# SZU-AdvTech-2022/232-Hierarchical-Density-based-Clustering-Using-Mapreduce

Hardware: AMD Instinct MI355X
Metric: points/sec end-to-end + mutual-reach distance evals/sec at 1/2/4/8 GPUs (higher is better)
Workload: dtype f64

## Files before the change

232-hierarchical-density-based-clustering-using-mapreduce_amd/csrc/flat.hip:

```cpp
#include <rocprim/device/device_scan.hpp>

#include <algorithm>
#include <chrono>
#include <numeric>

#include "common.hpp"
#include "internal.hpp"
#include "sort.hpp"
#include "ssort.hpp"

namespace hdb {

namespace {

constexpr int32_t NONE = INT32_MAX;
enum : int { FE_RANGE = 1, FE_NAN = 2, FE_CYCLE = 4, FE_ISOLATED = 8, FE_ROOTS = 16, FE_JUMP = 32 };

__device__ __forceinline__ uint32_t uf_prio(int32_t x, int64_t n) {
    uint32_t h = (uint32_t)x * 0x9E3779B1u;
    h ^= h >> 16;
    h *= 0x85EBCA6Bu;
    h ^= h >> 13;
    return (x >= n ? 0x80000000u : 0u) | (h >> 1);
}

struct __align__(16) LRec {
    int32_t uf, rootedge, csize, cmin;
};

__device__ __forceinline__ int32_t uf_ld(const int32_t *p) {
    return __hip_atomic_load(p, __ATOMIC_RELAXED, __HIP_MEMORY_SCOPE_AGENT);
}
__device__ __forceinline__ void uf_st(int32_t *p, int32_t v) {
    __hip_atomic_store(p, v, __ATOMIC_RELAXED, __HIP_MEMORY_SCOPE_AGENT);
}
__device__ __forceinline__ int32_t uf_find(LRec *lr, int32_t x) {
    int32_t *u = &lr->uf;
    while (true) {
        int32_t p = uf_ld(u + 4 * (int64_t)x);
        if (p == x) return x;
        int32_t g = uf_ld(u + 4 * (int64_t)p);
        if (g == p) return p;
        uf_st(u + 4 * (int64_t)x, g);
        x = g;
    }
}

__device__ __forceinline__ int32_t uf_unite(LRec *uf, int32_t a, int32_t b, int64_t n) {
    while (true) {
// ... 113 lines not shown
__global__ void fl_relabel_orig(const int32_t *__restrict__ pparent, const int32_t *__restrict__ eb, int64_t n,
                                int32_t *__restrict__ orig) {
    HDB_GRID_STRIDE(v, n) {
        const int32_t p = pparent[v];
        if (p == NONE) continue;
        orig[2 * (int64_t)p + (eb[p] == (int32_t)v ? 1 : 0)] = (int32_t)v;
    }
}
__global__ void fl_relabel(const int32_t *__restrict__ ea, const int32_t *__restrict__ eb,
                           const int32_t *__restrict__ pparent, int64_t m, int32_t *__restrict__ lab) {
    HDB_GRID_STRIDE(r, m) {
#pragma unroll
        for (int s = 0; s < 2; s++) {
            const int32_t v = s ? eb[r] : ea[r];
            const int32_t p = pparent[v];
            lab[2 * r + s] = 2 * p + (eb[p] == v ? 1 : 0);
        }
    }
}

__device__ __forceinline__ int64_t l_rank(int64_t i, int b) {
    return ((i >> b) << (b + 1)) | (i & ((int64_t(1) << b) - 1));
}

struct DC {
    int32_t *lab;
    LRec *lr;
    int32_t *stamp;
    int32_t *hooked;
    int32_t *parent;
    int32_t *esize;
    int32_t *eminid;
    const int32_t *orig;
    int64_t n, m;
};
__device__ __forceinline__ int32_t vid(const DC &c, int32_t x) { return c.orig ? c.orig[x] : x; }

__global__ void dc_init(DC c, int b, int j, int64_t nl) {
    HDB_GRID_STRIDE(i, nl) {
        int64_t r = l_rank(i, b);
        if (r >= c.m) continue;
#pragma unroll
        for (int s = 0; s < 2; s++) {
            int32_t x = c.lab[2 * r + s];
            c.lr[x] = LRec{x, -1, 0, NONE};
            c.stamp[x] = 2 * j;
        }
    }
}

__global__ void dc_unite(DC c, int b, int64_t nl, int *__restrict__ err) {
    HDB_GRID_STRIDE(i, nl) {
        int64_t r = l_rank(i, b);
        if (r >= c.m) continue;
        const int32_t h = uf_unite(c.lr, c.lab[2 * r], c.lab[2 * r + 1], c.n);
        c.hooked[r] = h;
        if (h < 0) atomicOr(err, FE_CYCLE);
    }
}

__device__ __forceinline__ int32_t wave_max(int32_t v) {
    for (int o = 32; o >= 1; o >>= 1) v = max(v, __shfl_xor(v, o));
    return v;
}
__device__ __forceinline__ int32_t wave_min(int32_t v) {
    for (int o = 32; o >= 1; o >>= 1) v = min(v, __shfl_xor(v, o));
    return v;
}
__device__ __forceinline__ int32_t wave_sum(int32_t v) {
    for (int o = 32; o >= 1; o >>= 1) v += __shfl_xor(v, o);
    return v;
}

constexpr int ROOT_TB = 256, ROOT_SLOTS = 512;
template <int TB, int SLOTS>
__global__ __launch_bounds__(TB) void dc_root(DC c, int b, int j, int64_t nl) {
    __shared__ int32_t skey[SLOTS], smax[SLOTS], ssum[SLOTS], smin[SLOTS];
    const int t = threadIdx.x;
    for (int64_t base = (int64_t)blockIdx.x * TB; base < nl; base += (int64_t)gridDim.x * TB) {
        for (int k = t; k < SLOTS; k += TB) {
            skey[k] = -1;
            smax[k] = -1;
            ssum[k] = 0;
            smin[k] = NONE;
        }
        __syncthreads();
        const int64_t i = base + t;
        const int64_t r = i < nl ? l_rank(i, b) : c.m;
        if (r < c.m) {
            const int32_t rep = uf_find(c.lr, c.lab[2 * r]);
            const int32_t x = c.hooked[r];
            c.hooked[r] = rep;
            const int32_t sz = x < 0 ? 0 : (x < c.n ? 1 : c.esize[x - c.n]);
            const int32_t mi = x < 0 ? NONE : (x < c.n ? vid(c, x) : c.eminid[x - c.n]);
            uint32_t h = uf_prio(rep, 0) & (SLOTS - 1);
            while (true) {
                int32_t k = atomicCAS(&skey[h], -1, rep);
                if (k == -1 || k == rep) break;
                h = (h + 1) & (SLOTS - 1);
            }
            atomicMax(&smax[h], (int32_t)r);
            if (sz) atomicAdd(&ssum[h], sz);
            if (mi != NONE) atomicMin(&smin[h], mi);
        }
        __syncthreads();
        for (int k = t; k < SLOTS; k += TB) {
            const int32_t rep = skey[k];
            if (rep < 0) continue;
            atomicMax(&c.lr[rep].rootedge, smax[k]);
            if (ssum[k]) atomicAdd(&c.lr[rep].csize, ssum[k]);
            if (smin[k] != NONE) atomicMin(&c.lr[rep].cmin, smin[k]);
        }
        __syncthreads();
    }
}

template <int TB, int SLOTS, int EPT>
__global__ __launch_bounds__(TB) void dc_root_multi(DC c, int b, int j, int64_t nl) {
    __shared__ int32_t skey[SLOTS], smax[SLOTS], ssum[SLOTS], smin[SLOTS];
    __shared__ int s_used;
    const int t = threadIdx.x;
    auto clear = [&]() {
        for (int k = t; k < SLOTS; k += TB) {
            skey[k] = -1;
            smax[k] = -1;
            ssum[k] = 0;
            smin[k] = NONE;
        }
        if (t == 0) s_used = 0;
    };
    auto flush = [&]() {
        for (int k = t; k < SLOTS; k += TB) {
            const int32_t rep = skey[k];
            if (rep < 0) continue;
            atomicMax(&c.lr[rep].rootedge, smax[k]);
            if (ssum[k]) atomicAdd(&c.lr[rep].csize, ssum[k]);
            if (smin[k] != NONE) atomicMin(&c.lr[rep].cmin, smin[k]);
        }
    };
    const int64_t per = (int64_t)TB * EPT;
    for (int64_t base = (int64_t)blockIdx.x * per; base < nl; base += (int64_t)gridDim.x * per) {
        clear();
        __syncthreads();
        for (int e = 0; e < EPT; e++) {
            const int64_t i = base + (int64_t)e * TB + t;
            const int64_t r = i < nl ? l_rank(i, b) : c.m;
            if (r < c.m) {
                const int32_t rep = uf_find(c.lr, c.lab[2 * r]);
                const int32_t x = c.hooked[r];
                c.hooked[r] = rep;
                const int32_t sz = x < 0 ? 0 : (x < c.n ? 1 : c.esize[x - c.n]);
                const int32_t mi = x < 0 ? NONE : (x < c.n ? vid(c, x) : c.eminid[x - c.n]);
                uint32_t h = uf_prio(rep, 0) & (SLOTS - 1);
                while (true) {
                    const int32_t k = atomicCAS(&skey[h], -1, rep);
                    if (k == -1) {
                        atomicAdd(&s_used, 1);
                        break;
                    }
                    if (k == rep) break;
                    h = (h + 1) & (SLOTS - 1);
                }
                atomicMax(&smax[h], (int32_t)r);
                if (sz) atomicAdd(&ssum[h], sz);
                if (mi != NONE) atomicMin(&smin[h], mi);
            }
            __syncthreads();
            if (e + 1 < EPT && s_used > SLOTS / 2 - TB) {
                flush();
                __syncthreads();
                clear();
                __syncthreads();
            }
        }
        flush();
        __syncthreads();
    }
}

__global__ void dc_root_direct(DC c, int b, int j, int64_t nl) {
    HDB_GRID_STRIDE(i, nl) {
        const int64_t r = l_rank(i, b);
        if (r >= c.m) continue;
        const int32_t rep = uf_find(c.lr, c.lab[2 * r]);
        const int32_t x = c.hooked[r];
        c.hooked[r] = rep;
        atomicMax(&c.lr[rep].rootedge, (int32_t)r);
        if (x >= 0) {
            atomicAdd(&c.lr[rep].csize, x < c.n ? 1 : c.esize[x - c.n]);
            atomicMin(&c.lr[rep].cmin, x < c.n ? vid(c, x) : c.eminid[x - c.n]);
        }
    }
}

__global__ void dc_link(DC c, int b, int j, int64_t nl) {
    HDB_GRID_STRIDE(i, nl) {
        int64_t r = l_rank(i, b);
        if (r >= c.m) continue;
        {
            const int32_t rep = c.hooked[r];
            const LRec q = c.lr[rep];
            if (q.rootedge == (int32_t)r) {
                c.esize[r] = q.csize + (rep < c.n ? 1 : c.esize[rep - c.n]);
                c.eminid[r] = min(q.cmin, rep < c.n ? vid(c, rep) : c.eminid[rep - c.n]);
            }
        }
        const int64_t u = r | (int64_t(1) << b);
        if (u >= c.m) continue;
#pragma unroll
        for (int s = 0; s < 2; s++) {
            int32_t x = c.lab[2 * u + s];
            if (c.stamp[x] == 2 * j) {
                const int32_t R = c.lr[uf_find(c.lr, x)].rootedge;
                if (uf_ld(c.parent + R) > (int32_t)u) atomicMin(&c.parent[R], (int32_t)u);
                c.lab[2 * u + s] = (int32_t)(c.n + R);
            }
        }
    }
}

template <int TB, int SLOTS, int EPT>
__global__ __launch_bounds__(TB) void dc_link_multi(DC c, int b, int j, int64_t nl) {
    __shared__ int32_t skey[SLOTS], smin[SLOTS];
    __shared__ int s_used;
    const int t = threadIdx.x;
    auto clear = [&]() {
        for (int k = t; k < SLOTS; k += TB) {
            skey[k] = -1;
            smin[k] = INT32_MAX;
        }
        if (t == 0) s_used = 0;
    };
    auto flush = [&]() {
        for (int k = t; k < SLOTS; k += TB) {
            const int32_t R = skey[k];
            if (R < 0) continue;
            if (uf_ld(c.parent + R) > smin[k]) atomicMin(&c.parent[R], smin[k]);
        }
    };
    const int64_t per = (int64_t)TB * EPT;
    for (int64_t base = (int64_t)blockIdx.x * per; base < nl; base += (int64_t)gridDim.x * per) {
        clear();
        __syncthreads();
        for (int e = 0; e < EPT; e++) {
            const int64_t i = base + (int64_t)e * TB + t;
            const int64_t r = i < nl ? l_rank(i, b) : c.m;
            if (r < c.m) {
                {
                    const int32_t rep = c.hooked[r];
                    const LRec q = c.lr[rep];
                    if (q.rootedge == (int32_t)r) {
                        c.esize[r] = q.csize + (rep < c.n ? 1 : c.esize[rep - c.n]);
                        c.eminid[r] = min(q.cmin, rep < c.n ? vid(c, rep) : c.eminid[rep - c.n]);
                    }
                }
                const int64_t u = r | (int64_t(1) << b);
                if (u < c.m) {
#pragma unroll
                    for (int s = 0; s < 2; s++) {
                        const int32_t x = c.lab[2 * u + s];
                        if (c.stamp[x] == 2 * j) {
                            const int32_t R = c.lr[uf_find(c.lr, x)].rootedge;
                            uint32_t h = uf_prio(R, 0) & (SLOTS - 1);
                            while (true) {
                                const int32_t k = atomicCAS(&skey[h], -1, R);
                                if (k == -1) {
                                    atomicAdd(&s_used, 1);
                                    break;
                                }
                                if (k == R) break;
                                h = (h + 1) & (SLOTS - 1);
                            }
                            atomicMin(&smin[h], (int32_t)u);
                            c.lab[2 * u + s] = (int32_t)(c.n + R);
                        }
                    }
                }
            }
            __syncthreads();
            if (e + 1 < EPT && s_used > SLOTS / 2 - 2 * TB) {
                flush();
                __syncthreads();
                clear();
                __syncthreads();
            }
        }
// ... 34 lines not shown
            c.hooked[r] = h;
            if (h < 0) e_cyc = 1;
        }
        dc_phase_sync();
        {
            int32_t *skey = tab, *smax = tab + RS, *ssum = tab + 2 * RS, *smin = tab + 3 * RS;
            auto clear = [&]() {
                for (int k = t; k < RS; k += TB) {
                    skey[k] = -1;
                    smax[k] = -1;
                    ssum[k] = 0;
                    smin[k] = NONE;
                }
                if (t == 0) s_used = 0;
            };
            auto flush = [&]() {
                for (int k = t; k < RS; k += TB) {
                    const int32_t rep = skey[k];
                    if (rep < 0) continue;
                    atomicMax(&c.lr[rep].rootedge, smax[k]);
                    if (ssum[k]) atomicAdd(&c.lr[rep].csize, ssum[k]);
                    if (smin[k] != NONE) atomicMin(&c.lr[rep].cmin, smin[k]);
                }
            };
            clear();
            __syncthreads();
            for (int64_t base = i0; base < i1; base += TB) {
                const int64_t i = base + t;
                if (i < i1) {
                    const int64_t r = l_rank(i, b);
                    const int32_t rep = uf_find(c.lr, c.lab[2 * r]);
                    const int32_t x = c.hooked[r];
                    c.hooked[r] = rep;
                    const int32_t sz = x < 0 ? 0 : (x < c.n ? 1 : c.esize[x - c.n]);
                    const int32_t mi = x < 0 ? NONE : (x < c.n ? vid(c, x) : c.eminid[x - c.n]);
                    uint32_t h = uf_prio(rep, 0) & (RS - 1);
                    while (true) {
                        const int32_t k = atomicCAS(&skey[h], -1, rep);
                        if (k == -1) {
                            atomicAdd(&s_used, 1);
                            break;
                        }
                        if (k == rep) break;
                        h = (h + 1) & (RS - 1);
                    }
                    atomicMax(&smax[h], (int32_t)r);
                    if (sz) atomicAdd(&ssum[h], sz);
                    if (mi != NONE) atomicMin(&smin[h], mi);
                }
                __syncthreads();
                if (base + TB < i1 && s_used > RS / 2 - TB) {
                    flush();
                    __syncthreads();
                    clear();
                    __syncthreads();
                }
            }
            flush();
        }
        dc_phase_sync();
        {
            int32_t *skey = tab, *smin = tab + KS;
            auto clear = [&]() {
                for (int k = t; k < KS; k += TB) {
                    skey[k] = -1;
                    smin[k] = INT32_MAX;
                }
                if (t == 0) s_used = 0;
            };
            auto flush = [&]() {
                for (int k = t; k < KS; k += TB) {
                    const int32_t R = skey[k];
                    if (R < 0) continue;
                    if (uf_ld(c.parent + R) > smin[k]) atomicMin(&c.parent[R], smin[k]);
                }
            };
            clear();
            __syncthreads();
            for (int64_t base = i0; base < i1; base += TB) {
                const int64_t i = base + t;
                if (i < i1) {
                    const int64_t r = l_rank(i, b);
                    {
                        const int32_t rep = c.hooked[r];
                        const LRec q = c.lr[rep];
                        if (q.rootedge == (int32_t)r) {
                            c.esize[r] = q.csize + (rep < c.n ? 1 : c.esize[rep - c.n]);
                            c.eminid[r] = min(q.cmin, rep < c.n ? vid(c, rep) : c.eminid[rep - c.n]);
                        }
                    }
                    const int64_t u = r | half;
                    if (u < c.m) {
#pragma unroll
                        for (int s = 0; s < 2; s++) {
                            const int32_t x = c.lab[2 * u + s];
                            if (c.stamp[x] == 2 * j) {
                                const int32_t R = c.lr[uf_find(c.lr, x)].rootedge;
                                uint32_t h = uf_prio(R, 0) & (KS - 1);
                                while (true) {
                                    const int32_t k = atomicCAS(&skey[h], -1, R);
                                    if (k == -1) {
                                        atomicAdd(&s_used, 1);
                                        break;
                                    }
                                    if (k == R) break;
                                    h = (h + 1) & (KS - 1);
                                }
                                atomicMin(&smin[h], (int32_t)u);
                                c.lab[2 * u + s] = (int32_t)(c.n + R);
                            }
                        }
                    }
                }
                __syncthreads();
                if (base + TB < i1 && s_used > KS / 2 - 2 * TB) {
                    flush();
                    __syncthreads();
                    clear();
                    __syncthreads();
                }
            }
// ... 17 lines not shown
        if (g == p) return p;
        ((volatile int32_t *)uf)[x] = g;
        x = g;
    }
}

template <int LB, int TB>
__global__ __launch_bounds__(TB) void dc_block(DC c, int *__restrict__ err) {
    using P = DcBlk<LB>;
    __shared__ int32_t key[P::HS], bsz[P::HS], bmn[P::HS];
    __shared__ int32_t uf[P::NL], re[P::NL], cs[P::NL], cm[P::NL];
    __shared__ int8_t stp[P::NL];
    __shared__ int16_t lab[2 * P::B];
    __shared__ int32_t esz[P::B], emn[P::B], lpar[P::B];
    __shared__ int16_t hk[P::B], rp[P::B];
    __shared__ int s_err;
    const int t = threadIdx.x;
    for (int64_t lo = (int64_t)blockIdx.x * P::B; lo < c.m; lo += (int64_t)gridDim.x * P::B) {
        const int cnt = (int)(c.m - lo < P::B ? c.m - lo : P::B);
        for (int k = t; k < P::HS; k += TB) key[k] = -1;
        for (int k = t; k < P::NL; k += TB) stp[k] = -1;
        for (int k = t; k < P::B; k += TB) {
            esz[k] = -1;
            lpar[k] = INT32_MAX;
        }
        if (t == 0) s_err = 0;
        __syncthreads();
        for (int k = t; k < 2 * cnt; k += TB) {
            const int32_t x = c.lab[2 * lo + k];
            uint32_t h = uf_prio(x, 0) & (P::HS - 1);
            while (true) {
                const int32_t old = atomicCAS(&key[h], -1, x);
                if (old == -1) {
                    bsz[h] = x < c.n ? 1 : c.esize[x - c.n];
                    bmn[h] = x < c.n ? vid(c, x) : c.eminid[x - c.n];
                    break;
                }
                if (old == x) break;
                h = (h + 1) & (P::HS - 1);
            }
            lab[k] = (int16_t)h;
        }
        __syncthreads();
        for (int b = LB - 1; b >= 0; b--) {
            const int half = 1 << b, nl = (P::B >> 1);
            for (int i = t; i < nl; i += TB) {
                const int k = ((i >> b) << (b + 1)) | (i & (half - 1));
                if (k >= cnt) continue;
#pragma unroll
                for (int s = 0; s < 2; s++) {
                    const int x = lab[2 * k + s];
                    uf[x] = x;
                    re[x] = -1;
                    cs[x] = x < P::HS ? bsz[x] : esz[x - P::HS];
                    cm[x] = x < P::HS ? bmn[x] : emn[x - P::HS];
                    stp[x] = (int8_t)b;
                }
            }
            __syncthreads();
            for (int i = t; i < nl; i += TB) {
                const int k = ((i >> b) << (b + 1)) | (i & (half - 1));
                if (k >= cnt) continue;
                int32_t a = lab[2 * k], d = lab[2 * k + 1], hooked = -1;
                while (true) {
                    a = lds_find(uf, a);
                    d = lds_find(uf, d);
                    if (a == d) break;
                    const uint32_t pa = uf_prio(a, P::HS), pd = uf_prio(d, P::HS);
                    if (pa < pd || (pa == pd && a < d)) {
                        const int32_t tt = a;
                        a = d;
                        d = tt;
                    }
                    if (atomicCAS(&uf[d], d, a) == d) {
                        hooked = d;
                        break;
                    }
                }
                if (hooked < 0) s_err = 1;
                hk[k] = (int16_t)hooked;
            }
            __syncthreads();
            for (int i = t; i < nl; i += TB) {
                const int k = ((i >> b) << (b + 1)) | (i & (half - 1));
                if (k >= cnt) continue;
                const int32_t rep = lds_find(uf, lab[2 * k]);
                rp[k] = (int16_t)rep;
                atomicMax(&re[rep], k);
                const int32_t x = hk[k];
                if (x >= 0) {
                    atomicAdd(&cs[rep], cs[x]);
                    atomicMin(&cm[rep], cm[x]);
                }
            }
            __syncthreads();
            for (int i = t; i < nl; i += TB) {
                const int k = ((i >> b) << (b + 1)) | (i & (half - 1));
                if (k >= cnt) continue;
                const int32_t rep = rp[k];
                if (re[rep] == k) {
                    esz[k] = cs[rep];
                    emn[k] = cm[rep];
                }
                const int u = k | half;
                if (u >= cnt) continue;
#pragma unroll
                for (int s = 0; s < 2; s++) {
                    const int x = lab[2 * u + s];
                    if (stp[x] == (int8_t)b) {
                        const int32_t R = re[lds_find(uf, x)];
                        atomicMin(&lpar[R], u);
                        lab[2 * u + s] = (int16_t)(P::HS + R);
                    }
                }
            }
            __syncthreads();
        }
        for (int k = t; k < cnt; k += TB) {
            if (esz[k] >= 0) {
                c.esize[lo + k] = esz[k];
                c.eminid[lo + k] = emn[k];
            }
            if (lpar[k] != INT32_MAX) c.parent[lo + k] = (int32_t)(lo + lpar[k]);
        }
        if (t == 0 && s_err) atomicOr(err, FE_CYCLE);
        __syncthreads();
    }
}

constexpr int LOC_LOG = 8, LOC_EDGES = 1 << LOC_LOG, LOC_SLOTS = 4 * LOC_EDGES;
__global__ __launch_bounds__(64) void dc_local(DC c, int *__restrict__ err) {
    __shared__ int32_t key[LOC_SLOTS], lsz[LOC_SLOTS], lmn[LOC_SLOTS];
    __shared__ int16_t luf[LOC_SLOTS], lre[LOC_SLOTS];
    __shared__ int16_t le[2 * LOC_EDGES];
    const int lane = threadIdx.x;
    for (int64_t lo = (int64_t)blockIdx.x * LOC_EDGES; lo < c.m; lo += (int64_t)gridDim.x * LOC_EDGES) {
        const int cnt = (int)(c.m - lo < LOC_EDGES ? c.m - lo : LOC_EDGES);
        for (int k = lane; k < LOC_SLOTS; k += 64) key[k] = -1;
        __syncthreads();
        for (int k = lane; k < 2 * cnt; k += 64) {
            const int32_t x = c.lab[2 * lo + k];
            uint32_t h = uf_prio(x, 0) & (LOC_SLOTS - 1);
            while (true) {
                const int32_t old = atomicCAS(&key[h], -1, x);
                if (old == -1) {
                    luf[h] = (int16_t)h;
                    lre[h] = -1;
                    lsz[h] = x < c.n ? 1 : c.esize[x - c.n];
                    lmn[h] = x < c.n ? vid(c, x) : c.eminid[x - c.n];
                    break;
                }
                if (old == x) break;
                h = (h + 1) & (LOC_SLOTS - 1);
            }
            le[k] = (int16_t)h;
        }
        __syncthreads();
        if (lane == 0) {
            auto find = [&](int x) {
                while (luf[x] != x) {
                    const int g = luf[luf[x]];
                    luf[x] = (int16_t)g;
                    x = g;
                }
                return x;
            };
            for (int k = 0; k < cnt; k++) {
                int a = find(le[2 * k]), b = find(le[2 * k + 1]);
                if (a == b) {
                    atomicOr(err, FE_CYCLE);
                    break;
                }
                if (lre[a] >= 0) c.parent[lo + lre[a]] = (int32_t)(lo + k);
                if (lre[b] >= 0) c.parent[lo + lre[b]] = (int32_t)(lo + k);
                if (lsz[a] < lsz[b]) {
                    const int t = a;
                    a = b;
                    b = t;
                }
                luf[b] = (int16_t)a;
                lsz[a] += lsz[b];
                lmn[a] = min(lmn[a], lmn[b]);
                lre[a] = (int16_t)k;
                c.esize[lo + k] = lsz[a];
                c.eminid[lo + k] = lmn[a];
            }
        }
        __syncthreads();
    }
}

__global__ void fl_tie_up(const int32_t *__restrict__ parent, const double *__restrict__ ew, int64_t m,
                          int32_t *__restrict__ up, int *__restrict__ err) {
    int e = 0;
    HDB_GRID_STRIDE(r, m) {
        int32_t p = parent[r];
        up[r] = (p != NONE && ew[p] == ew[r]) ? p : (int32_t)r;
        if (p == NONE && r != m - 1) e |= FE_ROOTS;
    }
    if (e) atomicOr(err, e);
}

__global__ void fl_jump(int32_t *__restrict__ up, int64_t m, const int *__restrict__ flag_prev,
                        int *__restrict__ flag_next) {
    if (flag_prev && *flag_prev == 0) return;
    int ch = 0;
    HDB_GRID_STRIDE(r, m) {
        int32_t p = up[r];
        bool moved = false;
#pragma unroll 1
        for (int it = 0; it < 2; it++) {
            const int32_t g = up[p];
            if (g == p) break;
            p = up[g];
            moved = true;
        }
        if (moved) {
            up[r] = p;
            ch = 1;
        }
    }
    flag_or(flag_next, ch);
// ... 943 lines not shown
                cur = c0;
                if (bt[cur] <= eps) {
                    int j = 0;
                    int32_t last = cur;
                    while (j < J) {
                        const int32_t a = anc[j * stride + cur];
                        if (!(bt[a] <= eps)) break;
                        last = a;
                        j++;
                    }
                    for (int jj = j - 2; jj >= 0; jj--) {
                        const int32_t a = anc[jj * stride + last];
                        if (bt[a] <= eps) last = a;
                    }
                    cur = anc[last];
                }
                const double pl = point_level[y], ee = pl > eps ? pl : eps;
                sc = ee == 0.0 ? 0.0 : 1.0 - ord_dec(em[cur]) / ee;
            }
        }
        if (tree_label) tree_label[i] = cur;
        if (labels) labels[i] = near[cur];
        if (scores) scores[i] = sc;
    }
    flag_or(err, e);
}

inline size_t fz_layout(int64_t m) { return (size_t)m * 24 + (size_t)m * 8 + 192 * 4; }

void throw_tree_errors(int e) {
    if (e & FE_CYCLE) HDB_THROW(HDB_EINVAL, "flat labels: the edges contain a cycle");
    if (e & FE_ROOTS) HDB_THROW(HDB_EINVAL, "flat labels: the edges are not a spanning tree");
    if (e & FE_JUMP) HDB_THROW(HDB_EDEVICE, "flat labels: pointer jumping did not converge in its launch budget");
}

}

static void flat_device_impl(hdb_ctx *ctx, const int32_t *va, const int32_t *vb, const double *w, int64_t ne,
                             int64_t n, int32_t mcs, int32_t *labels, int64_t *n_clusters, double *scores,
                             double *noise, const ClusterTreeOut *tree = nullptr) {
    if (n <= 0) {
        if (n_clusters) *n_clusters = 0;
        if (tree) *tree->n_tree = 0;
        return;
    }
    if (mcs < 2) HDB_THROW(HDB_EINVAL, "flat labels: minClSize must be >= 2");
    if (n >= (int64_t(1) << 30)) HDB_THROW(HDB_EINVAL, "flat labels: too many points");
    if (ne < 0) HDB_THROW(HDB_EINVAL, "bad arguments");
    hipStream_t st = ctx->stream;
    KernelTimer tt(ctx, "flat_labels");
    const int64_t m = n - 1;
    int64_t *pin = pinned_words(ctx) + PINNED_WORDS - 8;
    const int64_t mm = std::max<int64_t>(m, 1);
    const bool relabel = ctx->flat_relabel && m >= 1 && flat_relabel_fits(m);
    const int64_t nv = relabel ? 2 * mm : n;

    int32_t *keep, *pos, *ca, *cb, *ea, *eb, *orig, *pparent;
    double *cw, *ew;
    int64_t *words;
    DC dc;
    carve(ctx, A_FLAT0, [&](Carver &cv) {
        keep = cv.take<int32_t>(ne), pos = cv.take<int32_t>(ne);
        ca = cv.take<int32_t>(mm), cb = cv.take<int32_t>(mm);
        cw = cv.take<double>(mm);
        words = cv.take<int64_t>(4);
        ea = cv.take<int32_t>(mm), eb = cv.take<int32_t>(mm);
        ew = cv.take<double>(mm);
        dc.lab = cv.take<int32_t>(2 * mm);
        dc.lr = cv.take<LRec>(nv + mm);
        dc.stamp = cv.take<int32_t>(nv + mm);
        orig = cv.take<int32_t>(nv);
        dc.hooked = cv.take<int32_t>(mm);
        dc.parent = cv.take<int32_t>(mm);
        dc.esize = cv.take<int32_t>(mm);
        dc.eminid = cv.take<int32_t>(mm);
        pparent = cv.take<int32_t>(n);
    });
    int64_t *m_dev = words;
    int *err = (int *)(words + 1), *flags = (int *)(words + 2);
    dc.n = nv;
    dc.m = m;
    dc.orig = relabel ? orig : nullptr;

    HIP_CHECK(hipMemsetAsync(words, 0, sizeof(int64_t) * 4, st));
    if (ne > 0) {
        if (ne > INT32_MAX) HDB_THROW(HDB_EINVAL, "too many edges");
        hipLaunchKernelGGL(fl_mark, dim3(grid_for(ne)), dim3(256), 0, st, va, vb, w, ne, n, keep, err);
        exclusive_sum(ctx, A_FLAT_TMP, keep, pos, ne);
        hipLaunchKernelGGL(fl_compact, dim3(grid_for(ne)), dim3(256), 0, st, va, vb, w, ne, keep, pos, m, ca, cb, cw,
                           m_dev);
        hipLaunchKernelGGL(fl_order, dim3((unsigned)std::min<int64_t>(grid_for(ne) / 4 + 1, 256)), dim3(1024), 0, st,
                           cw, m_dev, flags);
    }
    HIP_CHECK(hipMemcpyAsync(pin, words, sizeof(int64_t) * 3, hipMemcpyDeviceToHost, st));
    HIP_CHECK(hipStreamSynchronize(st));
    const int64_t m_got = pin[0];
    const int e0 = (int)pin[1], order = (int)pin[2];
    if (e0 & FE_RANGE) HDB_THROW(HDB_EINVAL, "flat labels: vertex id out of range");
    if (e0 & FE_NAN) HDB_THROW(HDB_EINVAL, "flat labels: NaN edge weight");
    if (m_got != m) HDB_THROW(HDB_EINVAL, "flat labels: the edges are not a spanning tree");
    if (m == 0) {
        if (labels) HIP_CHECK(hipMemsetAsync(labels, 0, sizeof(int32_t), st));
        if (scores) HIP_CHECK(hipMemsetAsync(scores, 0, sizeof(double), st));
        if (noise) HIP_CHECK(hipMemsetAsync(noise, 0, sizeof(double), st));
        if (n_clusters) *n_clusters = 0;
        if (tree) {
            *tree->n_tree = 1;
            if (tree->cap < 1) HDB_THROW(HDB_EINVAL, "cluster tree: capacity 0 is below the 1 clusters of the tree");
            hipLaunchKernelGGL(ct_single, dim3(1), dim3(64), 0, st, *tree);
            HIP_CHECK(hipGetLastError());
            HIP_CHECK(hipStreamSynchronize(st));
        }
        return;
    }
    const int g = grid_for(m);
    const int32_t *perm = nullptr;
    int desc = !(order & 1);
    if (desc == 0 && (order & 2)) {
        double *k1, *k2;
        int32_t *i1, *i2;
        carve(ctx, A_FLAT1, [&](Carver &cv) {
            k1 = cv.take<double>(m), k2 = cv.take<double>(m);
            i1 = cv.take<int32_t>(m), i2 = cv.take<int32_t>(m);
        });
        hipLaunchKernelGGL(fl_sort_keys, dim3(g), dim3(256), 0, st, cw, m, k1, i1);
        sort_pairs(ctx, A_FLAT_TMP, k1, k2, i1, i2, m, 0, 64);
        perm = i2;
    }
    hipLaunchKernelGGL(fl_rank, dim3(g), dim3(256), 0, st, ca, cb, cw, m, desc, perm, ea, eb, ew, dc.lab, dc.parent);
    hipLaunchKernelGGL(fill_i32, dim3(grid_for(nv + m)), dim3(256), 0, st, dc.stamp, nv + m, -1);
    hipLaunchKernelGGL(fill_i32, dim3(grid_for(n)), dim3(256), 0, st, pparent, n, NONE);
    hipLaunchKernelGGL(fl_point_parent, dim3(g), dim3(256), 0, st, ea, eb, m, pparent);
    if (relabel) {
        hipLaunchKernelGGL(fl_relabel_orig, dim3(grid_for(n)), dim3(256), 0, st, pparent, eb, n, orig);
        hipLaunchKernelGGL(fl_relabel, dim3(g), dim3(256), 0, st, ea, eb, pparent, m, dc.lab);
    }

    int J = 0;
    while ((int64_t(1) << J) <= m) J++;
    const int LB = ctx->flat_block_log >= 8 && ctx->flat_block_log <= 10 ? ctx->flat_block_log : LOC_LOG;
    const int LM = ctx->flat_mid_log > LB ? std::max(LB, std::min(ctx->flat_mid_log, J)) : LB;
    ctx->stats["flat_global_depths"] = std::max(0, J - LM);
    ctx->stats["flat_mid_depths"] = LM - LB;
    for (int j = 0; j < J - LM; j++) {
        const int b = J - 1 - j;
        const int64_t blk = int64_t(1) << (b + 1), half = int64_t(1) << b;
        const int64_t nl = (m / blk) * half + std::min(m % blk, half);
        const int gl = grid_for(nl);
        hipLaunchKernelGGL(dc_init, dim3(gl), dim3(256), 0, st, dc, b, j, nl);
        hipLaunchKernelGGL(dc_unite, dim3(gl), dim3(256), 0, st, dc, b, nl, err);
        const bool deep = j >= ctx->flat_deep_depth;
        switch (deep ? ctx->flat_deep_root : ctx->flat_root_variant) {
        case 1: hipLaunchKernelGGL((dc_root<1024, 4096>), dim3((unsigned)ceil_div(nl, 1024)), dim3(1024), 0, st, dc, b, j, nl); break;
        case 2: hipLaunchKernelGGL(dc_root_direct, dim3(gl), dim3(256), 0, st, dc, b, j, nl); break;
        case 3: hipLaunchKernelGGL((dc_root_multi<1024, 4096, 4>), dim3((unsigned)ceil_div(nl, 4096)), dim3(1024), 0, st, dc, b, j, nl); break;
        case 4: hipLaunchKernelGGL((dc_root_multi<1024, 8192, 4>), dim3((unsigned)ceil_div(nl, 4096)), dim3(1024), 0, st, dc, b, j, nl); break;
        case 5: hipLaunchKernelGGL((dc_root_multi<512, 4096, 4>), dim3((unsigned)ceil_div(nl, 2048)), dim3(512), 0, st, dc, b, j, nl); break;
        default: hipLaunchKernelGGL((dc_root<ROOT_TB, ROOT_SLOTS>), dim3(gl), dim3(ROOT_TB), 0, st, dc, b, j, nl);
        }
        if ((deep ? ctx->flat_deep_link : ctx->flat_link_variant) == 1)
            hipLaunchKernelGGL((dc_link_multi<1024, 8192, 2>), dim3((unsigned)ceil_div(nl, 2048)), dim3(1024), 0, st, dc,
                               b, j, nl);
        else
            hipLaunchKernelGGL(dc_link, dim3(gl), dim3(256), 0, st, dc, b, j, nl);
    }
    if (LM > LB)
        hipLaunchKernelGGL(dc_mid<1024>, dim3((unsigned)ceil_div(m, int64_t(1) << LM)), dim3(1024), 0, st, dc, J, LM, LB,
                           err);
    const unsigned nblk = (unsigned)std::min<int64_t>(ceil_div(m, int64_t(1) << LB), 65536);
    switch (ctx->flat_block_log) {
    case 8: hipLaunchKernelGGL((dc_block<8, 128>), dim3(nblk), dim3(128), 0, st, dc, err); break;
    case 9: hipLaunchKernelGGL((dc_block<9, 256>), dim3(nblk), dim3(256), 0, st, dc, err); break;
    case 10: hipLaunchKernelGGL((dc_block<10, 512>), dim3(nblk), dim3(512), 0, st, dc, err); break;
    default: hipLaunchKernelGGL(dc_local, dim3(nblk), dim3(64), 0, st, dc, err);
    }

    int32_t *top = (int32_t *)dc.lr, *pnode = top + (n + m), *nvalid = pnode + (n + m), *vsum = nvalid + (n + m),
            *is_start = dc.stamp;
    int32_t *cs, *cid, *seg, *cpar, *cminid, *clab, *csz, *kstart, *kids, *pnodes, *poff, *ssel, *Kp, *rc, *rl, *mlist,
        *llist, *mk, *rk;
    uint64_t *key1, *key2, *jw, *tw, *lw;
    double *val1, *val2, *stab, *cpv, *rs, *mpre, *postv;
    int *jflags;
    unsigned long long *groot;
    char *fz;
    const size_t fz_bytes = fz_layout(m);
    carve(ctx, A_FLAT1, [&](Carver &cv) {
        cs = cv.take<int32_t>(m), cid = cv.take<int32_t>(m);
        key1 = cv.take<uint64_t>(m), key2 = cv.take<uint64_t>(m);
        val1 = cv.take<double>(m), val2 = cv.take<double>(m);
        seg = cv.take<int32_t>(m);
        stab = cv.take<double>(m);
        cpar = cv.take<int32_t>(m), cminid = cv.take<int32_t>(m), clab = cv.take<int32_t>(m);
        jflags = cv.take<int32_t>(64);
        groot = cv.take<unsigned long long>(1);
        csz = cv.take<int32_t>(m), kstart = cv.take<int32_t>(m), kids = cv.take<int32_t>(m);
        pnodes = cv.take<int32_t>(m), poff = cv.take<int32_t>(m);
        ssel = cv.take<int32_t>(m), Kp = cv.take<int32_t>(m), rc = cv.take<int32_t>(m);
        rl = cv.take<int32_t>(m), mlist = cv.take<int32_t>(m), llist = cv.take<int32_t>(m);
        jw = cv.take<uint64_t>(m), tw = cv.take<uint64_t>(m);
        cpv = cv.take<double>(m);
        lw = cv.take<uint64_t>(m);
        rs = cv.take<double>(m), mpre = cv.take<double>(m), postv = cv.take<double>(m);
        fz = cv.take<char>(fz_bytes);
        mk = cv.take<int32_t>(n), rk = cv.take<int32_t>(n);
    });
    int32_t *nch = (int32_t *)fz, *kcur = nch + m, *plen = kcur + m, *maxld = plen + m;
// ... 284 lines not shown
```

Measured before the change: 182.0 million.

## Contract MST chains before divide-and-conquer Kruskal dendrogram build

```diff
diff --git a/232-hierarchical-density-based-clustering-using-mapreduce_amd/csrc/flat.hip b/232-hierarchical-density-based-clustering-using-mapreduce_amd/csrc/flat.hip
--- a/232-hierarchical-density-based-clustering-using-mapreduce_amd/csrc/flat.hip
+++ b/232-hierarchical-density-based-clustering-using-mapreduce_amd/csrc/flat.hip
@@ -1,4 +1,5 @@
 #include <rocprim/device/device_scan.hpp>
+#include <rocprim/device/device_scan_by_key.hpp>
 
 #include <algorithm>
 #include <chrono>
@@ -14,7 +15,8 @@
 namespace {
 
 constexpr int32_t NONE = INT32_MAX;
-enum : int { FE_RANGE = 1, FE_NAN = 2, FE_CYCLE = 4, FE_ISOLATED = 8, FE_ROOTS = 16, FE_JUMP = 32 };
+enum : int { FE_RANGE = 1, FE_NAN = 2, FE_CYCLE = 4, FE_ISOLATED = 8, FE_ROOTS = 16, FE_JUMP = 32, FE_PASS = 64 };
+constexpr int64_t FLAT_CONTRACT_MIN_M = int64_t(1) << 18;
 
 __device__ __forceinline__ uint32_t uf_prio(int32_t x, int64_t n) {
     uint32_t h = (uint32_t)x * 0x9E3779B1u;
@@ -194,9 +196,21 @@
     int32_t *esize;
     int32_t *eminid;
     const int32_t *orig;
+    const int32_t *wv = nullptr, *mv = nullptr;
+    const int32_t *wl = nullptr, *ml = nullptr;
     int64_t n, m;
 };
 __device__ __forceinline__ int32_t vid(const DC &c, int32_t x) { return c.orig ? c.orig[x] : x; }
+__device__ __forceinline__ int32_t lab_size(const DC &c, int32_t x) {
+    if (x < c.n) return c.wv ? c.wv[x] : 1;
+    return c.esize[x - c.n];
+}
+__device__ __forceinline__ int32_t lab_min(const DC &c, int32_t x) {
+    if (x < c.n) return c.mv ? c.mv[x] : vid(c, x);
+    return c.eminid[x - c.n];
+}
+__device__ __forceinline__ int32_t edge_size(const DC &c, int64_t r) { return c.wl ? c.wl[r] : 0; }
+__device__ __forceinline__ int32_t edge_min(const DC &c, int64_t r) { return c.ml ? c.ml[r] : NONE; }
 
 __global__ void dc_init(DC c, int b, int j, int64_t nl) {
     HDB_GRID_STRIDE(i, nl) {
@@ -253,8 +267,8 @@
             const int32_t rep = uf_find(c.lr, c.lab[2 * r]);
             const int32_t x = c.hooked[r];
             c.hooked[r] = rep;
-            const int32_t sz = x < 0 ? 0 : (x < c.n ? 1 : c.esize[x - c.n]);
-            const int32_t mi = x < 0 ? NONE : (x < c.n ? vid(c, x) : c.eminid[x - c.n]);
+            const int32_t sz = (x < 0 ? 0 : lab_size(c, x)) + edge_size(c, r);
+            const int32_t mi = min(x < 0 ? NONE : lab_min(c, x), edge_min(c, r));
             uint32_t h = uf_prio(rep, 0) & (SLOTS - 1);
             while (true) {
                 int32_t k = atomicCAS(&skey[h], -1, rep);
@@ -311,8 +325,8 @@
                 const int32_t rep = uf_find(c.lr, c.lab[2 * r]);
                 const int32_t x = c.hooked[r];
                 c.hooked[r] = rep;
-                const int32_t sz = x < 0 ? 0 : (x < c.n ? 1 : c.esize[x - c.n]);
-                const int32_t mi = x < 0 ? NONE : (x < c.n ? vid(c, x) : c.eminid[x - c.n]);
+                const int32_t sz = (x < 0 ? 0 : lab_size(c, x)) + edge_size(c, r);
+                const int32_t mi = min(x < 0 ? NONE : lab_min(c, x), edge_min(c, r));
                 uint32_t h = uf_prio(rep, 0) & (SLOTS - 1);
                 while (true) {
                     const int32_t k = atomicCAS(&skey[h], -1, rep);
@@ -349,8 +363,12 @@
         c.hooked[r] = rep;
         atomicMax(&c.lr[rep].rootedge, (int32_t)r);
         if (x >= 0) {
-            atomicAdd(&c.lr[rep].csize, x < c.n ? 1 : c.esize[x - c.n]);
-            atomicMin(&c.lr[rep].cmin, x < c.n ? vid(c, x) : c.eminid[x - c.n]);
+            atomicAdd(&c.lr[rep].csize, lab_size(c, x));
+            atomicMin(&c.lr[rep].cmin, lab_min(c, x));
+        }
+        if (c.wl) {
+            atomicAdd(&c.lr[rep].csize, c.wl[r]);
+            atomicMin(&c.lr[rep].cmin, c.ml[r]);
         }
     }
 }
@@ -363,8 +381,8 @@
             const int32_t rep = c.hooked[r];
             const LRec q = c.lr[rep];
             if (q.rootedge == (int32_t)r) {
-                c.esize[r] = q.csize + (rep < c.n ? 1 : c.esize[rep - c.n]);
-                c.eminid[r] = min(q.cmin, rep < c.n ? vid(c, rep) : c.eminid[rep - c.n]);
+                c.esize[r] = q.csize + lab_size(c, rep);
+                c.eminid[r] = min(q.cmin, lab_min(c, rep));
             }
         }
         const int64_t u = r | (int64_t(1) << b);
@@ -412,8 +430,8 @@
                     const int32_t rep = c.hooked[r];
                     const LRec q = c.lr[rep];
                     if (q.rootedge == (int32_t)r) {
-                        c.esize[r] = q.csize + (rep < c.n ? 1 : c.esize[rep - c.n]);
-                        c.eminid[r] = min(q.cmin, rep < c.n ? vid(c, rep) : c.eminid[rep - c.n]);
+                        c.esize[r] = q.csize + lab_size(c, rep);
+                        c.eminid[r] = min(q.cmin, lab_min(c, rep));
                     }
                 }
                 const int64_t u = r | (int64_t(1) << b);
@@ -514,8 +532,8 @@
                     const int32_t rep = uf_find(c.lr, c.lab[2 * r]);
                     const int32_t x = c.hooked[r];
                     c.hooked[r] = rep;
-                    const int32_t sz = x < 0 ? 0 : (x < c.n ? 1 : c.esize[x - c.n]);
-                    const int32_t mi = x < 0 ? NONE : (x < c.n ? vid(c, x) : c.eminid[x - c.n]);
+                    const int32_t sz = (x < 0 ? 0 : lab_size(c, x)) + edge_size(c, r);
+                    const int32_t mi = min(x < 0 ? NONE : lab_min(c, x), edge_min(c, r));
                     uint32_t h = uf_prio(rep, 0) & (RS - 1);
                     while (true) {
                         const int32_t k = atomicCAS(&skey[h], -1, rep);
@@ -567,8 +585,8 @@
                         const int32_t rep = c.hooked[r];
                         const LRec q = c.lr[rep];
                         if (q.rootedge == (int32_t)r) {
-                            c.esize[r] = q.csize + (rep < c.n ? 1 : c.esize[rep - c.n]);
-                            c.eminid[r] = min(q.cmin, rep < c.n ? vid(c, rep) : c.eminid[rep - c.n]);
+                            c.esize[r] = q.csize + lab_size(c, rep);
+                            c.eminid[r] = min(q.cmin, lab_min(c, rep));
                         }
                     }
                     const int64_t u = r | half;
@@ -652,8 +670,8 @@
             while (true) {
                 const int32_t old = atomicCAS(&key[h], -1, x);
                 if (old == -1) {
-                    bsz[h] = x < c.n ? 1 : c.esize[x - c.n];
-                    bmn[h] = x < c.n ? vid(c, x) : c.eminid[x - c.n];
+                    bsz[h] = lab_size(c, x);
+                    bmn[h] = lab_min(c, x);
                     break;
                 }
                 if (old == x) break;
@@ -712,6 +730,10 @@
                     atomicAdd(&cs[rep], cs[x]);
                     atomicMin(&cm[rep], cm[x]);
                 }
+                if (c.wl) {
+                    atomicAdd(&cs[rep], c.wl[lo + k]);
+                    atomicMin(&cm[rep], c.ml[lo + k]);
+                }
             }
             __syncthreads();
             for (int i = t; i < nl; i += TB) {
@@ -766,8 +788,8 @@
                 if (old == -1) {
                     luf[h] = (int16_t)h;
                     lre[h] = -1;
-                    lsz[h] = x < c.n ? 1 : c.esize[x - c.n];
-                    lmn[h] = x < c.n ? vid(c, x) : c.eminid[x - c.n];
+                    lsz[h] = lab_size(c, x);
+                    lmn[h] = lab_min(c, x);
                     break;
                 }
                 if (old == x) break;
@@ -799,8 +821,8 @@
                     b = t;
                 }
                 luf[b] = (int16_t)a;
-                lsz[a] += lsz[b];
-                lmn[a] = min(lmn[a], lmn[b]);
+                lsz[a] += lsz[b] + edge_size(c, lo + k);
+                lmn[a] = min(min(lmn[a], lmn[b]), edge_min(c, lo + k));
                 lre[a] = (int16_t)k;
                 c.esize[lo + k] = lsz[a];
                 c.eminid[lo + k] = lmn[a];
@@ -808,6 +830,196 @@
         }
         __syncthreads();
     }
+}
+
+struct __align__(8) CMin {
+    int32_t s, mn;
+};
+struct CMinOp {
+    __host__ __device__ CMin operator()(const CMin &a, const CMin &b) const {
+        return CMin{a.s + b.s, a.mn < b.mn ? a.mn : b.mn};
+    }
+};
+
+struct KA {
+    const int32_t *ea, *eb, *pparent;
+    int32_t *up;
+    uint64_t *f2, *p2;
+    CMin *cv;
+    int32_t *ev;
+    int32_t *proot, *ppos;
+    int32_t *a0;
+    int32_t *arank;
+    int32_t *lab0;
+    int32_t *anc;
+    int32_t *wv, *mv, *wl, *ml, *lfirst;
+    int32_t *exm;
+    uint32_t *kin, *kout;
+    int32_t *vin, *vout;
+    CMin *sin, *sout;
+    int64_t *cnt;
+    int64_t m, cap;
+};
+
+__global__ void ka_classify(KA k) {
+    HDB_GRID_STRIDE(e, k.m) {
+        const int32_t u = k.ea[e], v = k.eb[e], mu = k.pparent[u], mv = k.pparent[v];
+        const int cu = mu == (int32_t)e, cv = mv == (int32_t)e, c = cu + cv;
+        k.f2[e] = (uint64_t)(c == 0) | ((uint64_t)(c == 2) << 32);
+        k.up[e] = c == 1 ? (cu ? mv : mu) : (int32_t)e;
+        k.cv[e] = CMin{c, min(cu ? u : NONE, cv ? v : NONE)};
+        if (c == 2 && k.proot) k.proot[min(u, v)] = 1;
+    }
+}
+
+__global__ void ka_find(KA k) {
+    HDB_GRID_STRIDE(e, k.m) {
+        if (e == k.m - 1) {
+            const uint64_t t = k.p2[e] + k.f2[e];
+            k.cnt[0] = (int64_t)(t & 0xffffffffu);
+            k.cnt[1] = (int64_t)(t >> 32);
+        }
+        if (k.f2[e] & 1) continue;
+        const int32_t r = up_find(k.up, (int32_t)e);
+        k.ev[e] = k.ppos ? k.ppos[min(k.ea[r], k.eb[r])] : (int32_t)(k.p2[r] >> 32);
+    }
+}
+
+__global__ void ka_alpha(KA k, DC c) {
+    HDB_GRID_STRIDE(e, k.m) {
+        if (!(k.f2[e] & 1)) continue;
+        const int64_t a = (int64_t)(k.p2[e] & 0xffffffffu);
+        if (a >= k.cap) continue;
+        k.arank[a] = (int32_t)e;
+        c.parent[a] = NONE;
+#pragma unroll
+        for (int s = 0; s < 2; s++) {
+            const int32_t V = k.ev[k.pparent[s ? k.eb[e] : k.ea[e]]];
+            c.lab[2 * a + s] = V;
+            k.lab0[2 * a + s] = V;
+            atomicMin(&k.a0[V], (int32_t)a);
+        }
+    }
+}
+
+__global__ void ka_init(KA k, DC c) {
+    HDB_GRID_STRIDE(i, 2 * k.cap + 1) {
+        c.stamp[i] = -1;
+        if (i <= k.cap) k.a0[i] = NONE;
+        if (i < k.cap) {
+            k.wl[i] = 0;
+            k.ml[i] = NONE;
+            k.lfirst[i] = NONE;
+        }
+    }
+}
+
+__global__ void ka_anc0(KA k, DC c) {
+    HDB_GRID_STRIDE(a, c.m + 1) {
+        const int32_t p = a < c.m ? c.parent[a] : NONE;
+        k.anc[a] = p == NONE ? (int32_t)c.m : p;
+    }
+}
+
+__global__ void ka_keys(KA k, int64_t ma, int64_t na, int rows) {
+    HDB_GRID_STRIDE(e, k.m) {
+        uint32_t key = (uint32_t)(2 * ma + 1);
+        if (!(k.f2[e] & 1)) {
+            const int32_t V = k.ev[e], a0v = k.a0[V], ap = (int32_t)(k.p2[e] & 0xffffffffu);
+            key = (uint32_t)V;
+            if (a0v != NONE && ap > a0v) {
+                int32_t b = a0v;
+                for (int j = rows - 1; j >= 0; j--) {
+                    const int32_t t = k.anc[(int64_t)j * (ma + 1) + b];
+                    if (t < ap) b = t;
+                }
+                key = (uint32_t)(na + b);
+            }
+        }
+        k.kin[e] = key;
+        k.vin[e] = (int32_t)e;
+    }
+}
+
+__global__ void ka_gather(KA k) {
+    HDB_GRID_STRIDE(i, k.m) k.sin[i] = k.cv[k.vout[i]];
+}
+
+__global__ void ka_runs(KA k, int64_t ma, int64_t na) {
+    const int64_t cnt = k.m - ma;
+    HDB_GRID_STRIDE(i, cnt) {
+        const uint32_t key = k.kout[i];
+        if (i == 0 || k.kout[i - 1] != key)
+            if (key >= na) k.lfirst[key - na] = k.vout[i];
+        if (i == cnt - 1 || k.kout[i + 1] != key) {
+            const CMin t = k.sout[i];
+            if (key < na) {
+                k.wv[key] = t.s;
+                k.mv[key] = t.mn;
+            } else {
+                k.wl[key - na] = t.s;
+                k.ml[key - na] = t.mn;
+            }
+        }
+    }
+}
+
+__global__ void ka_reset(KA k, DC c) {
+    HDB_GRID_STRIDE(i, c.n + c.m) {
+        c.stamp[i] = -1;
+        if (i < c.m) {
+            c.parent[i] = NONE;
+            k.exm[i] = NONE;
+            c.lab[2 * i] = k.lab0[2 * i];
+            c.lab[2 * i + 1] = k.lab0[2 * i + 1];
+        }
+    }
+}
+
+__global__ void ka_exmin(KA k, DC c) {
+    HDB_GRID_STRIDE(i, c.n + c.m) {
+        if (i < c.m) {
+            const int32_t p = k.anc[i];
+            if (p != (int32_t)c.m) atomicMin(&k.exm[p], c.eminid[i]);
+        } else {
+            const int32_t a = k.a0[i - c.m];
+            if (a != NONE) atomicMin(&k.exm[a], k.mv[i - c.m]);
+        }
+    }
+}
+
+__global__ void ka_write(KA k, DC c, int32_t *__restrict__ parent, int32_t *__restrict__ esize,
+                         int32_t *__restrict__ eminid, int *__restrict__ err) {
+    const int64_t ma = c.m, na = c.n, cnt = k.m - ma;
+    int bad = 0;
+    auto rank_of = [&](int32_t a) { return a == NONE || a == (int32_t)ma ? NONE : k.arank[a]; };
+    HDB_GRID_STRIDE(i, k.m) {
+        const int32_t e = k.vout[i];
+        if (i >= cnt) {
+            const int64_t a = i - cnt;
+            esize[e] = c.esize[a] - k.wl[a];
+            eminid[e] = k.exm[a];
+            const int32_t pa = k.anc[a], f = k.lfirst[a];
+            parent[e] = f != NONE ? f : rank_of(pa);
+            if (c.parent[a] != (pa == (int32_t)ma ? NONE : pa)) bad = FE_PASS;
+            continue;
+        }
+        const uint32_t key = k.kout[i];
+        const CMin t = k.sout[i];
+        int32_t base = 0, bmin = NONE, last;
+        if (key < na) {
+            last = rank_of(k.a0[key]);
+        } else {
+            const int64_t b = key - na;
+            base = c.esize[b] - k.wl[b];
+            bmin = k.exm[b];
+            last = rank_of(k.anc[b]);
+        }
+        esize[e] = base + t.s;
+        eminid[e] = min(bmin, t.mn);
+        parent[e] = i + 1 < cnt && k.kout[i + 1] == key ? k.vout[i + 1] : last;
+    }
+    flag_or(err, bad);
 }
 
 __global__ void fl_tie_up(const int32_t *__restrict__ parent, const double *__restrict__ ew, int64_t m,
@@ -1817,6 +2029,7 @@
     if (e & FE_CYCLE) HDB_THROW(HDB_EINVAL, "flat labels: the edges contain a cycle");
     if (e & FE_ROOTS) HDB_THROW(HDB_EINVAL, "flat labels: the edges are not a spanning tree");
     if (e & FE_JUMP) HDB_THROW(HDB_EDEVICE, "flat labels: pointer jumping did not converge in its launch budget");
+    if (e & FE_PASS) HDB_THROW(HDB_EDEVICE, "flat labels: the two passes over the contracted tree disagree");
 }
 
 }
@@ -1844,11 +2057,17 @@
     double *cw, *ew;
     int64_t *words;
     DC dc;
+    const bool contract = m >= FLAT_CONTRACT_MIN_M;
+    const int64_t acap = m / 2 + 1;
+    int arows = 1;
+    while ((int64_t(1) << arows) < acap) arows++;
+    DC da{};
+    KA ka{};
     carve(ctx, A_FLAT0, [&](Carver &cv) {
         keep = cv.take<int32_t>(ne), pos = cv.take<int32_t>(ne);
         ca = cv.take<int32_t>(mm), cb = cv.take<int32_t>(mm);
         cw = cv.take<double>(mm);
-        words = cv.take<int64_t>(4);
+        words = cv.take<int64_t>(6);
         ea = cv.take<int32_t>(mm), eb = cv.take<int32_t>(mm);
         ew = cv.take<double>(mm);
         dc.lab = cv.take<int32_t>(2 * mm);
@@ -1860,6 +2079,23 @@
         dc.esize = cv.take<int32_t>(mm);
         dc.eminid = cv.take<int32_t>(mm);
         pparent = cv.take<int32_t>(n);
+        if (!contract) return;
+        da.lab = cv.take<int32_t>(2 * acap), ka.lab0 = cv.take<int32_t>(2 * acap);
+        da.lr = cv.take<LRec>(2 * acap + 1);
+        da.stamp = cv.take<int32_t>(2 * acap + 1);
+        da.hooked = cv.take<int32_t>(acap), da.parent = cv.take<int32_t>(acap);
+        da.esize = cv.take<int32_t>(acap), da.eminid = cv.take<int32_t>(acap);
+        ka.a0 = cv.take<int32_t>(acap + 1), ka.arank = cv.take<int32_t>(acap);
+        ka.wv = cv.take<int32_t>(acap + 1), ka.mv = cv.take<int32_t>(acap + 1);
+        ka.wl = cv.take<int32_t>(acap), ka.ml = cv.take<int32_t>(acap), ka.lfirst = cv.take<int32_t>(acap);
+        ka.exm = cv.take<int32_t>(acap);
+        ka.anc = cv.take<int32_t>((acap + 1) * arows);
+        ka.up = cv.take<int32_t>(mm), ka.ev = cv.take<int32_t>(mm);
+        ka.f2 = cv.take<uint64_t>(mm), ka.p2 = cv.take<uint64_t>(mm);
+        ka.cv = cv.take<CMin>(mm), ka.sin = cv.take<CMin>(mm), ka.sout = cv.take<CMin>(mm);
+        ka.kin = cv.take<uint32_t>(mm), ka.kout = cv.take<uint32_t>(mm);
+        ka.vin = cv.take<int32_t>(mm), ka.vout = cv.take<int32_t>(mm);
+        ka.proot = cv.take<int32_t>(n), ka.ppos = cv.take<int32_t>(n);
     });
     int64_t *m_dev = words;
     int *err = (int *)(words + 1), *flags = (int *)(words + 2);
@@ -1913,51 +2149,107 @@
         perm = i2;
     }
     hipLaunchKernelGGL(fl_rank, dim3(g), dim3(256), 0, st, ca, cb, cw, m, desc, perm, ea, eb, ew, dc.lab, dc.parent);
-    hipLaunchKernelGGL(fill_i32, dim3(grid_for(nv + m)), dim3(256), 0, st, dc.stamp, nv + m, -1);
+    if (!contract) hipLaunchKernelGGL(fill_i32, dim3(grid_for(nv + m)), dim3(256), 0, st, dc.stamp, nv + m, -1);
     hipLaunchKernelGGL(fill_i32, dim3(grid_for(n)), dim3(256), 0, st, pparent, n, NONE);
     hipLaunchKernelGGL(fl_point_parent, dim3(g), dim3(256), 0, st, ea, eb, m, pparent);
-    if (relabel) {
+    if (relabel && !contract) {
         hipLaunchKernelGGL(fl_relabel_orig, dim3(grid_for(n)), dim3(256), 0, st, pparent, eb, n, orig);
         hipLaunchKernelGGL(fl_relabel, dim3(g), dim3(256), 0, st, ea, eb, pparent, m, dc.lab);
     }
 
-    int J = 0;
-    while ((int64_t(1) << J) <= m) J++;
-    const int LB = ctx->flat_block_log >= 8 && ctx->flat_block_log <= 10 ? ctx->flat_block_log : LOC_LOG;
-    const int LM = ctx->flat_mid_log > LB ? std::max(LB, std::min(ctx->flat_mid_log, J)) : LB;
-    ctx->stats["flat_global_depths"] = std::max(0, J - LM);
-    ctx->stats["flat_mid_depths"] = LM - LB;
-    for (int j = 0; j < J - LM; j++) {
-        const int b = J - 1 - j;
-        const int64_t blk = int64_t(1) << (b + 1), half = int64_t(1) << b;
-        const int64_t nl = (m / blk) * half + std::min(m % blk, half);
-        const int gl = grid_for(nl);
-        hipLaunchKernelGGL(dc_init, dim3(gl), dim3(256), 0, st, dc, b, j, nl);
-        hipLaunchKernelGGL(dc_unite, dim3(gl), dim3(256), 0, st, dc, b, nl, err);
-        const bool deep = j >= ctx->flat_deep_depth;
-        switch (deep ? ctx->flat_deep_root : ctx->flat_root_variant) {
-        case 1: hipLaunchKernelGGL((dc_root<1024, 4096>), dim3((unsigned)ceil_div(nl, 1024)), dim3(1024), 0, st, dc, b, j, nl); break;
-        case 2: hipLaunchKernelGGL(dc_root_direct, dim3(gl), dim3(256), 0, st, dc, b, j, nl); break;
-        case 3: hipLaunchKernelGGL((dc_root_multi<1024, 4096, 4>), dim3((unsigned)ceil_div(nl, 4096)), dim3(1024), 0, st, dc, b, j, nl); break;
-        case 4: hipLaunchKernelGGL((dc_root_multi<1024, 8192, 4>), dim3((unsigned)ceil_div(nl, 4096)), dim3(1024), 0, st, dc, b, j, nl); break;
-        case 5: hipLaunchKernelGGL((dc_root_multi<512, 4096, 4>), dim3((unsigned)ceil_div(nl, 2048)), dim3(512), 0, st, dc, b, j, nl); break;
-        default: hipLaunchKernelGGL((dc_root<ROOT_TB, ROOT_SLOTS>), dim3(gl), dim3(ROOT_TB), 0, st, dc, b, j, nl);
-        }
-        if ((deep ? ctx->flat_deep_link : ctx->flat_link_variant) == 1)
-            hipLaunchKernelGGL((dc_link_multi<1024, 8192, 2>), dim3((unsigned)ceil_div(nl, 2048)), dim3(1024), 0, st, dc,
-                               b, j, nl);
-        else
-            hipLaunchKernelGGL(dc_link, dim3(gl), dim3(256), 0, st, dc, b, j, nl);
-    }
-    if (LM > LB)
-        hipLaunchKernelGGL(dc_mid<1024>, dim3((unsigned)ceil_div(m, int64_t(1) << LM)), dim3(1024), 0, st, dc, J, LM, LB,
-                           err);
-    const unsigned nblk = (unsigned)std::min<int64_t>(ceil_div(m, int64_t(1) << LB), 65536);
-    switch (ctx->flat_block_log) {
-    case 8: hipLaunchKernelGGL((dc_block<8, 128>), dim3(nblk), dim3(128), 0, st, dc, err); break;
-    case 9: hipLaunchKernelGGL((dc_block<9, 256>), dim3(nblk), dim3(256), 0, st, dc, err); break;
-    case 10: hipLaunchKernelGGL((dc_block<10, 512>), dim3(nblk), dim3(512), 0, st, dc, err); break;
-    default: hipLaunchKernelGGL(dc_local, dim3(nblk), dim3(64), 0, st, dc, err);
+    auto kruskal_dc = [&](const DC &c) {
+        const int64_t m = c.m;
+        int J = 0;
+        while ((int64_t(1) << J) <= m) J++;
+        const int LB = ctx->flat_block_log >= 8 && ctx->flat_block_log <= 10 ? ctx->flat_block_log : LOC_LOG;
+        const int LM = ctx->flat_mid_log > LB ? std::max(LB, std::min(ctx->flat_mid_log, J)) : LB;
+        ctx->stats["flat_global_depths"] = std::max(0, J - LM);
+        ctx->stats["flat_mid_depths"] = LM - LB;
+        if (m == 0) return;
+        for (int j = 0; j < J - LM; j++) {
+            const int b = J - 1 - j;
+            const int64_t blk = int64_t(1) << (b + 1), half = int64_t(1) << b;
+            const int64_t nl = (m / blk) * half + std::min(m % blk, half);
+            const int gl = grid_for(nl);
+            hipLaunchKernelGGL(dc_init, dim3(gl), dim3(256), 0, st, c, b, j, nl);
+            hipLaunchKernelGGL(dc_unite, dim3(gl), dim3(256), 0, st, c, b, nl, err);
+            const bool deep = j >= ctx->flat_deep_depth;
+            switch (deep ? ctx->flat_deep_root : ctx->flat_root_variant) {
+            case 1: hipLaunchKernelGGL((dc_root<1024, 4096>), dim3((unsigned)ceil_div(nl, 1024)), dim3(1024), 0, st, c, b, j, nl); break;
+            case 2: hipLaunchKernelGGL(dc_root_direct, dim3(gl), dim3(256), 0, st, c, b, j, nl); break;
+            case 3: hipLaunchKernelGGL((dc_root_multi<1024, 4096, 4>), dim3((unsigned)ceil_div(nl, 4096)), dim3(1024), 0, st, c, b, j, nl); break;
+            case 4: hipLaunchKernelGGL((dc_root_multi<1024, 8192, 4>), dim3((unsigned)ceil_div(nl, 4096)), dim3(1024), 0, st, c, b, j, nl); break;
+            case 5: hipLaunchKernelGGL((dc_root_multi<512, 4096, 4>), dim3((unsigned)ceil_div(nl, 2048)), dim3(512), 0, st, c, b, j, nl); break;
+            default: hipLaunchKernelGGL((dc_root<ROOT_TB, ROOT_SLOTS>), dim3(gl), dim3(ROOT_TB), 0, st, c, b, j, nl);
+            }
+            if ((deep ? ctx->flat_deep_link : ctx->flat_link_variant) == 1)
+                hipLaunchKernelGGL((dc_link_multi<1024, 8192, 2>), dim3((unsigned)ceil_div(nl, 2048)), dim3(1024), 0, st,
+                                   c, b, j, nl);
+            else
+                hipLaunchKernelGGL(dc_link, dim3(gl), dim3(256), 0, st, c, b, j, nl);
+        }
+        if (LM > LB)
+            hipLaunchKernelGGL(dc_mid<1024>, dim3((unsigned)ceil_div(m, int64_t(1) << LM)), dim3(1024), 0, st, c, J, LM,
+                               LB, err);
+        const unsigned nblk = (unsigned)std::min<int64_t>(ceil_div(m, int64_t(1) << LB), 65536);
+        switch (ctx->flat_block_log) {
+        case 8: hipLaunchKernelGGL((dc_block<8, 128>), dim3(nblk), dim3(128), 0, st, c, err); break;
+        case 9: hipLaunchKernelGGL((dc_block<9, 256>), dim3(nblk), dim3(256), 0, st, c, err); break;
+        case 10: hipLaunchKernelGGL((dc_block<10, 512>), dim3(nblk), dim3(512), 0, st, c, err); break;
+        default: hipLaunchKernelGGL(dc_local, dim3(nblk), dim3(64), 0, st, c, err);
+        }
+    };
+    ctx->stats["flat_contract"] = contract ? 1 : 0;
+    ctx->stats["flat_alpha_edges"] = 0;
+    if (!contract) {
+        kruskal_dc(dc);
+    } else {
+        ka.ea = ea, ka.eb = eb, ka.pparent = pparent;
+        ka.cnt = words + 4;
+        ka.m = m, ka.cap = acap;
+        if (!relabel) {
+            HIP_CHECK(hipMemsetAsync(ka.proot, 0, sizeof(int32_t) * n, st));
+        } else {
+            ka.proot = ka.ppos = nullptr;
+        }
+        hipLaunchKernelGGL(ka_init, dim3(grid_for(2 * acap + 1)), dim3(256), 0, st, ka, da);
+        hipLaunchKernelGGL(ka_classify, dim3(g), dim3(256), 0, st, ka);
+        exclusive_sum(ctx, A_FLAT_TMP, ka.f2, ka.p2, m);
+        if (!relabel) exclusive_sum(ctx, A_FLAT_TMP, ka.proot, ka.ppos, n);
+        hipLaunchKernelGGL(ka_find, dim3(g), dim3(256), 0, st, ka);
+        hipLaunchKernelGGL(ka_alpha, dim3(g), dim3(256), 0, st, ka, da);
+        HIP_CHECK(hipMemcpyAsync(pin, ka.cnt, sizeof(int64_t) * 2, hipMemcpyDeviceToHost, st));
+        HIP_CHECK(hipStreamSynchronize(st));
+        const int64_t ma = pin[0], na = pin[1];
+        if (ma != na - 1 || ma >= acap) HDB_THROW(HDB_EINVAL, "flat labels: the edges contain a cycle");
+        ctx->stats["flat_alpha_edges"] = ma;
+        da.n = na;
+        da.m = ma;
+        kruskal_dc(da);
+        int rows = 0;
+        while ((int64_t(1) << rows) < ma) rows++;
+        const int ga = grid_for(ma + 1);
+        hipLaunchKernelGGL(ka_anc0, dim3(ga), dim3(256), 0, st, ka, da);
+        for (int j = 1; j < rows; j++)
+            hipLaunchKernelGGL(lc_double, dim3(ga), dim3(256), 0, st, ka.anc + (j - 1) * (ma + 1), ka.anc + j * (ma + 1),
+                               (int32_t)ma);
+        hipLaunchKernelGGL(ka_keys, dim3(g), dim3(256), 0, st, ka, ma, na, rows);
+        int bits = 1;
+        while ((int64_t(1) << bits) < 2 * ma + 2) bits++;
+        sort_pairs(ctx, A_FLAT_TMP, ka.kin, ka.kout, ka.vin, ka.vout, m, 0, bits);
+        hipLaunchKernelGGL(ka_gather, dim3(g), dim3(256), 0, st, ka);
+        with_tmp(ctx, A_FLAT_TMP, [&](void *tmp, size_t &b) {
+            return rocprim::inclusive_scan_by_key(tmp, b, ka.kout, ka.sin, ka.sout, (size_t)m, CMinOp(),
+                                                  rocprim::equal_to<uint32_t>(), st);
+        });
+        hipLaunchKernelGGL(ka_runs, dim3(g), dim3(256), 0, st, ka, ma, na);
+        if (ma > 0) {
+            hipLaunchKernelGGL(ka_reset, dim3(grid_for(na + ma)), dim3(256), 0, st, ka, da);
+            da.wv = ka.wv, da.mv = ka.mv, da.wl = ka.wl, da.ml = ka.ml;
+            kruskal_dc(da);
+            hipLaunchKernelGGL(ka_exmin, dim3(grid_for(na + ma)), dim3(256), 0, st, ka, da);
+        }
+        hipLaunchKernelGGL(ka_write, dim3(g), dim3(256), 0, st, ka, da, dc.parent, dc.esize, dc.eminid, err);
     }
 
     int32_t *top = (int32_t *)dc.lr, *pnode = top + (n + m), *nvalid = pnode + (n + m), *vsum = nvalid + (n + m),
```

Measured after the change: 200.7 million (median of 6 runs). 10.3% higher.
